# masafumiendo/benchnav

Measured on AMD Instinct MI355X. Metric: MPPI solve-steps/sec (K=1024,T=50,256x256 map), higher is better.
Workload: dtype f32

## Files before the change

### benchnav_amd/csrc/mppi_capi.cpp

```cpp
#include "../../include/benchnav_mppi.h"
#include "mppi_kernels.h"
#include "astar_dwa.h"

#include <algorithm>
#include <atomic>
#include <cmath>
#include <chrono>
#include <cstdarg>
#include <cstdio>
#include <cstdlib>
#include <cstring>
#include <cerrno>
#include <sys/stat.h>
#include <fcntl.h>
#include <sys/file.h>
#include <unistd.h>
#include <dlfcn.h>
#include <hsa/hsa.h>
#include <hsa/hsa_ext_amd.h>
#include <rccl/rccl.h>
#include <map>
#include <mutex>
#include <numeric>
#include <string>
#include <vector>

namespace {

constexpr int kProfGroup = 10;
bool wave_kernel_is_faster(const bn::SolveParams &p, size_t resident_role_wgs, int n_cus)
{
    const double W = (double)p.B * (p.nblk + 1), R = (double)std::max<size_t>(resident_role_wgs, 1), rows = std::max(0, p.nblk - 16);
    const double role = (4.5 + 0.19 * p.T + 0.3 * rows) * (1.0 + 0.175 * std::min(W, R) / std::max(n_cus, 1)) * std::max(1.0, W / R);
    const double gain = (rows == 0 && p.T >= 20) ? 0.93 : 1.0;
    const double wave = gain * (3.3 + 0.44 * p.T + 0.37 * rows) * (1.0 + 1.5 * W / (24.0 * std::max(n_cus, 1)));
    return wave < role;
}
thread_local std::string g_last_error;

#ifdef BN_EXPERIMENTS
inline const char *exp_env(const char *name) { return std::getenv(name); }
#else
inline const char *exp_env(const char *) { return nullptr; }
#endif

int fail(int code, const char *fmt, ...)
{
    char buf[512];
    va_list ap;
    va_start(ap, fmt);
    vsnprintf(buf, sizeof buf, fmt, ap);
    va_end(ap);
    g_last_error = buf;
    return code;
}

#define BN_HIP(expr)                                                                         \
    do {                                                                                     \
        hipError_t e_ = (expr);                                                              \
        if (e_ != hipSuccess) {                                                              \
            (void)hipGetLastError();    \
            return fail(BN_ERR_HIP, "%s failed: %s (%s:%d)", #expr, hipGetErrorString(e_),  \
                        __FILE__, __LINE__);                                                 \
        }                                                                                    \
    } while (0)

bool is_pow2_float(float v)
{
    int ex;
    return v > 0.0f && std::isfinite(v) && std::frexp(v, &ex) == 0.5f;
}

std::mutex g_overlap_mu;
std::map<int, bn_mppi *> g_overlap_owner;
std::map<int, std::vector<bn_mppi *>> g_handles;
std::atomic<int> g_overlap_owners{0};
std::map<int, int> g_overlap_lock_fd;
// ... 54 lines not shown
    hipStream_t xstream[kMaxStreams - 1] = {};
    std::vector<hipStream_t> parked;
    hipEvent_t ev_fork = nullptr, ev_join[kMaxStreams - 1] = {};
    hipEvent_t ev_guard[kMaxStreams] = {};
    unsigned long long *d_flags = nullptr;
    bool role_overlap = false;
    unsigned long long *d_gran[kSlots] = {};
    float *d_Xalt[kMaxStreams - 1] = {}, *d_Ualt[kMaxStreams - 1] = {};
    unsigned long long pub[kSlots] = {};
    unsigned long long tails = 0;
    bool prev_published = false;
    bool overlap_used = false;
    bool overlap_off = false;
    int *h_err = nullptr, *d_err = nullptr;
    unsigned long long *h_mail = nullptr, *d_mail = nullptr;
    float *d_mean_snap = nullptr;
    float *d_state_snaps = nullptr;
    size_t snap_cap = 0;
    size_t snap_slot = 0;
    bool arm_state_snap = false;
    struct BatchRec { int32_t n; const float *states; const float *eps; bn_noise_kind noise; int32_t eps_ring; int64_t eps_stride; bool episode; const float *z; };
    std::vector<BatchRec> journal;
    bool journal_lost = false;
    bool arm_snap = false;
    bool replaying = false, last_batch_overlapped = false;
    uint64_t journal_solves0 = 0, recoveries = 0;
    struct OvTune { double best[2] = {0, 0}, last[2] = {0, 0}, ema[2] = {0, 0}; int chosen = 0, explore = 0, slow_run = 0; uint64_t windows[2] = {0, 0}, since_explore = 0, switches = 0; } tune;
    struct OvSample { bool valid = false; std::chrono::steady_clock::time_point t{}; uint32_t prog = 0, enq = 0; } ov_sample;
    int run_mode = 0;
    float *self_out_copy = nullptr;
    const float *inline_state = nullptr;
    bool self_tail_launched = false;
    bool self_used = false;
    bool self_off = false;
    bool hp_enabled = false;
    hipStream_t hp_stream[2] = {};
    hipEvent_t hp_ev[2] = {};
    bool hp_unordered = false;
    int hp_unordered_q = 0;
    unsigned long long *h_req = nullptr, *d_req = nullptr;
    unsigned long long *req_bar = nullptr;
    unsigned long long *d_req_dev = nullptr;
    uint32_t hp_seq = 0;
    bool hp_armed = false;
    uint32_t hp_tag = 0;
    int hp_slot = 0, hp_q = 0, hp_xidx = 0;
    uint32_t hp_posted_tag = 0;
    float hp_posted_state[3] = {};
    float *hp_posted_out = nullptr;
    bool hp_skip_check = false;
    int hp_redo_q = -1;
    float hp_prev_state[3] = {};
    bool hp_gran_valid = false;
    int hp_extra = 2;
    int x_idx = 0;
    int hp_next_q = 0;
    std::chrono::steady_clock::time_point hp_armed_at{};
    int hp_polls = 25000;
    bool lat_kernel = false;
    bool wave_kernel = false;
    bool shard_pending = false;
    void *shard_comm = nullptr;
    int shard_world = 0, shard_rank = 0;
    bool shard_prepared = false;
    bool shard_inplace = false;
    float *d_gathered = nullptr;
// ... 304 lines not shown
    BN_HIP(hipStreamSynchronize(h->stream));
    h->recoveries += 1;
    (void)fail(BN_OK, "warning: an overlapped launch gave up waiting for its predecessor's partials; %zu batch(es) were re-run on one "
                      "stream (results are valid now; this handle no longer overlaps its launches)", recs.size());
    return BN_OK;
}

int settle_overlap(bn_mppi *h, bool synced)
{
    if (!h->overlap_used || h->replaying) return BN_OK;
    if (__atomic_load_n(h->h_err, __ATOMIC_ACQUIRE) == 0) {
        if (synced) {
            bool idle = true;
            for (int q = 0; idle && q + 1 < h->n_streams; ++q) idle = hipStreamQuery(h->xstream[q]) == hipSuccess;
            (void)hipGetLastError();
            if (idle) { h->overlap_used = false; h->journal.clear(); h->journal_lost = false; }
        }
        return BN_OK;
    }
    return recover_overlap(h);
}

int sync_checked(bn_mppi *h)
{
    BN_HIP(hipStreamSynchronize(h->stream));
    if (h->overlap_used)
        for (int q = 0; q + 1 < h->n_streams; ++q)
            if (h->xstream[q]) BN_HIP(hipStreamSynchronize(h->xstream[q]));
    return settle_overlap(h, true);
}

int self_check(bn_mppi *h)
{
    if (!h->self_used || h->overlap_used || h->replaying) return BN_OK;
    if (__atomic_load_n(h->h_err, __ATOMIC_ACQUIRE) == 0) return BN_OK;
    BN_HIP(hipStreamSynchronize(h->stream));
    BN_HIP(hipMemset(h->d_flags, 0, ((kSlots + 1) * (size_t)h->p.B + 3) * bn::kFlagStride * sizeof(unsigned long long)));
    for (int q = 0; q < kSlots; ++q) h->pub[q] = 0;
    h->tails = 0;
    *h->h_err = 0;
    h->self_used = false;
    h->self_off = true;
    return fail(BN_ERR_HIP, "the tail of a one-launch solve gave up waiting for the rollout workgroups of its own launch: the outputs of solve %llu "
                            "are invalid (solve again); this handle goes back to two launches per synchronous solve",
                (unsigned long long)h->solves - 1);
}

int settle_point(bn_mppi *h)
{
    hp_cancel(h);
    h->hp_gran_valid = false;
    if (int rc = self_check(h)) return rc;
    if (!h->overlap_used || h->replaying) return BN_OK;
    if (int rc = flush_tail(h)) return rc;
    return sync_checked(h);
}

void tune_record(bn_mppi *h, int mode, double us)
{
    bn_mppi::OvTune &t = h->tune;
    t.last[mode] = us;
    t.ema[mode] = t.ema[mode] == 0 ? us : t.ema[mode] + (us - t.ema[mode]) / 8;
    if (us >= 0.7 * t.ema[mode] && (t.best[mode] == 0 || us < t.best[mode])) t.best[mode] = us;
    t.windows[mode] += 1;
    if (mode == t.chosen) {
        t.since_explore += 1;
// ... 534 lines not shown
static int order_behind_foreign_overlap(bn_mppi *h, hipStream_t st)
{
    std::lock_guard<std::mutex> lock(g_overlap_mu);
    auto it = g_overlap_owner.find(h->cfg.device_id);
    if (it == g_overlap_owner.end() || it->second == h || !it->second) return BN_OK;
    bn_mppi *o = it->second;
    bool busy = false;
    for (int q = 0; q < o->n_streams; ++q) {
        const hipStream_t os = q ? o->xstream[q - 1] : o->stream;
        if (os == st || (q && !os)) continue;
        if (hipStreamQuery(os) == hipSuccess) continue;
        busy = true;
        if (!o->ev_guard[q]) continue;
        BN_HIP(hipEventRecord(o->ev_guard[q], os));
        BN_HIP(hipStreamWaitEvent(st, o->ev_guard[q], 0));
    }
    (void)hipGetLastError();
    if (!busy) { g_overlap_owner.erase(it); g_overlap_owners.store((int)g_overlap_owner.size(), std::memory_order_relaxed); }
    return BN_OK;
}

namespace {
int guard_foreign_overlap(bn_mppi *h)
{
    if (h->last_batch_overlapped || g_overlap_owners.load(std::memory_order_relaxed) == 0) return BN_OK;
    return order_behind_foreign_overlap(h, h->stream);
}
}

static inline bool lone_self_redo(const bn_mppi *h, bool self_tail, bool overlap)
{
    return h->hp_redo_q >= 0 && self_tail && !overlap && h->lat_kernel && !h->in_episode && !h->tail_pending && !h->replaying && !h->self_off &&
           !(h->cfg.flags & BN_FLAG_NO_PIPELINE);
}

static int solve_impl(bn_mppi_t *h, const float *states, bn_mem_kind states_where, const float *eps, bn_noise_kind noise,
                      bool shard_rollout, bool overlap = false, hipStream_t on_stream = nullptr, int alt_buffers = 0, bool self_tail = false)
{
    if (!h) return fail(BN_ERR_INVALID, "null handle");
    if (!states) return fail(BN_ERR_INVALID, "states is null");
    if (!h->map_set || !h->goal_set) return fail(BN_ERR_STATE, "set_map and set_goal must precede solve");
    if ((noise == BN_NOISE_PHILOX) != (eps == nullptr))
        return fail(BN_ERR_INVALID, "eps must be NULL exactly when noise == BN_NOISE_PHILOX");
    BN_BIND(h);
    hp_cancel(h);
    h->hp_gran_valid = false;
    if (!overlap && g_overlap_owners.load(std::memory_order_relaxed) > 0) {
        if (int rc = order_behind_foreign_overlap(h, on_stream ? on_stream : h->stream)) return rc;
    }

    bn::SolveParams p = h->p;
    const size_t B = p.B, K = p.K, T = p.T;
    h->map_epoch_at_solve = h->map_epoch;
    if (h->d_flags && (h->overlap_used || !h->journal.empty()))
        p.err_dev = reinterpret_cast<int *>(h->d_flags + ((kSlots + 1) * B + 2) * bn::kFlagStride);
    if (states_where == BN_MEM_DEVICE) {
        p.state = states;
    } else {
        if (h->solves) BN_HIP(hipStreamSynchronize(h->stream));
        std::memcpy(h->h_pinned, states, B * 3 * 4);
        BN_HIP(hipMemcpyAsync(h->d_state, h->h_pinned, B * 3 * 4, hipMemcpyHostToDevice, h->stream));
        p.state = h->d_state;
    }
    bn::EpsMode mode = bn::kEpsPhilox;
    switch (noise) {
    case BN_NOISE_PHILOX: break;
// ... 95 lines not shown
            h->self_tail_launched = true;
            h->prev_published = false;
            h->hp_gran_valid = p.gran != nullptr;
            h->x_idx = 0;
        } else
        if ((h->lat_kernel || h->role_overlap) && overlap) {
            p.flag_part = h->d_flags;
            p.err = h->d_err; p.err_dev = reinterpret_cast<int *>(h->d_flags + ((kSlots + 1) * B + 2) * bn::kFlagStride);
            if (h->arm_snap) { p.mean_snap = h->d_mean_snap; h->arm_snap = false; }
            p.cur_slot = cur3; p.prev_slot = prev3;
            p.wait_part = h->pub[prev3];
            p.gran = p.lat_kernel ? h->d_gran[cur3] : nullptr;
            if (alt_buffers) {
                if (h->d_Xalt[alt_buffers - 1]) p.X = h->d_Xalt[alt_buffers - 1];
                if (h->d_Ualt[alt_buffers - 1] && p.U) p.U = h->d_Ualt[alt_buffers - 1];
            }
            p.overlap = (h->prev_published && p.have_prev) ? 1 : 0;
            p.gran_prev = (p.overlap && p.lat_kernel) ? h->d_gran[prev3] : nullptr;
            if (on_stream) st = on_stream;
            if (p.overlap) h->overlap_used = true;
            h->pub[cur3] += (unsigned long long)p.nblk;
            h->prev_published = true;
            if (self_tail && p.lat_kernel && !h->in_episode) {
                p.self_tail = 1;
                p.wait_part_self = h->pub[cur3];
                p.wait_tail_self = h->tails;
                h->tails += 1;
            }
        } else {
            h->prev_published = false;
        }
        p.aux_prio = (!p.wave_kernel && (size_t)p.B * (p.nblk + 1) > h->resident_wgs) ? 1 : 0;
        if (!p.wave_kernel && !p.store_u) p.U = nullptr;
        if (p.self_tail) BN_HIP(bn::launch_rollout_lat_self(p, mode, st));
        else BN_HIP(bn::launch_rollout(p, mode, st));
        if (st != h->stream && lone_self) {
            BN_HIP(hipEventRecord(h->hp_ev[h->hp_redo_q], st));
            BN_HIP(hipStreamWaitEvent(h->stream, h->hp_ev[h->hp_redo_q], 0));
        }
        if (prof_grouped) h->prof_in_group = (h->prof_in_group + 1) % kProfGroup;
        h->solves += 1;
        h->x_idx = 0;
        h->tail_pending = !p.self_tail;
        if (p.self_tail) h->prev_published = false;
        if (lone_self) h->last_batch_overlapped = false;
        return BN_OK;
    }
    if (!(h->ticket_overlap && overlap && !shard_rollout)) h->prev_published = false;
    p.have_prev = 0;
    p.mean_from_part = 0;
    p.tail_solve = p.solve;
    if (p.slip_on && !h->slip_std_set) return fail(BN_ERR_STATE, "bn_mppi_set_slip_std must precede solve in sampled-slip mode");
    if (h->ticket_mode && !shard_rollout) {
        p.have_prev = h->tail_pending ? 1 : 0;
        p.tail_merged = 1;
        p.tail_solve = p.solve - 1;
        p.ustar_cur = h->d_ustar2[cur3]; p.stats_cur = h->d_stats2[cur3];
        p.ustar_prev = h->d_ustar2[prev3]; p.stats_prev = h->d_stats2[prev3];
        p.ticket = h->d_ticket;
        hipStream_t st = h->stream;
        p.flag_tail = h->d_flags + kSlots * B * bn::kFlagStride;
        if (p.have_prev) { p.wait_tail = h->tails; h->tails += 1; }
        if (h->ticket_overlap && overlap) {
            p.flag_part = h->d_flags;
            p.err = h->d_err; p.err_dev = reinterpret_cast<int *>(h->d_flags + ((kSlots + 1) * B + 2) * bn::kFlagStride);
            if (h->arm_snap) { p.mean_snap = h->d_mean_snap; h->arm_snap = false; }
            p.cur_slot = cur3; p.prev_slot = prev3;
            p.wait_part = h->pub[prev3];
            if (alt_buffers) {
                if (h->d_Xalt[alt_buffers - 1]) p.X = h->d_Xalt[alt_buffers - 1];
                if (h->d_Ualt[alt_buffers - 1] && p.U) p.U = h->d_Ualt[alt_buffers - 1];
            }
            p.overlap = (h->prev_published && p.have_prev) ? 1 : 0;
            if (on_stream) st = on_stream;
            if (p.overlap) h->overlap_used = true;
            h->pub[cur3] += 1;
            h->prev_published = true;
        }
        if (p.slip_on) BN_HIP(bn::launch_rollout_sampled(p, mode, st));
        else BN_HIP(bn::launch_rollout(p, mode, st));
        if (prof_grouped) h->prof_in_group = (h->prof_in_group + 1) % kProfGroup;
        h->solves += 1;
        h->tail_pending = true;
        return BN_OK;
    }
    if (shard_rollout && h->shard_inplace) p.part = h->d_gathered + (size_t)h->shard_rank * p.nblk * (2 + 2 * T);
    if (p.slip_on) {
        BN_HIP(bn::launch_rollout_sampled(p, mode, h->stream));
    } else {
        if (h->slow_path) p.wave_kernel = 1;
        else if (!p.store_u) p.U = nullptr;
        BN_HIP(bn::launch_rollout(p, mode, h->stream));
    }
    if (prof) BN_HIP(hipEventRecord(ev[1], h->stream));
    if (shard_rollout) {
        if (prof) BN_HIP(hipEventRecord(ev[2], h->stream));
        h->solves += 1;
        h->tail_pending = false;
        h->shard_pending = true;
        return BN_OK;
    }
    p.state = p.state_copy;
    BN_HIP(bn::launch_finish(p, h->stream));
    if (prof) BN_HIP(hipEventRecord(ev[2], h->stream));
    h->solves += 1;
    h->tail_pending = false;
    return BN_OK;
}

int bn_mppi_solve_async(bn_mppi_t *h, const float *states, bn_mem_kind states_where, const float *eps,
                        bn_noise_kind noise)
{
    if (h && !h->replaying && !h->journal.empty()) {
        h->last_batch_overlapped = false;
        journal_arm_states(h);
        journal_push(h, bn_mppi::BatchRec{1, states, eps, noise, 1, 0, false, nullptr}, states_where == BN_MEM_DEVICE && noise != BN_NOISE_HOST_KT2);
    }
    return solve_impl(h, states, states_where, eps, noise, false);
}

#ifdef BN_TIMING
struct HpClock { const char *name; long long ns = 0, n = 0; };
static HpClock g_hpc[6] = {{"post: request words"}, {"post: hipStreamWaitEvent"}, {"prelaunch: checks + ack"}, {"prelaunch: kernel launch"}, {"prelaunch: hipEventRecord"}, {"self_check + bind"}};
struct HpTick { int i; std::chrono::steady_clock::time_point t0 = std::chrono::steady_clock::now();
// ... 1287 lines not shown
```

### benchnav_amd/csrc/mppi_kernels.h

```cpp
#pragma once
#include <hip/hip_runtime.h>
#include <stdint.h>

namespace bn {

constexpr int kRolloutsPerBlock = 64;
constexpr int kRolloutThreads = 320;
constexpr int kChunk = 4;
constexpr int kWaveParkSteps = 30;
constexpr int kUPad = 65;
constexpr int kWideFinishThreads = 1024;
constexpr int kFinishThreads = kRolloutThreads;

enum EpsMode : int { kEpsPhilox = 0, kEpsKT2 = 1, kEpsT2K = 2 };

struct SolveParams {
    int K, T, G, B;
    int nblk;
    int Kp;
    int WN;
    int reach;
    int spec_extra;
    int map_stride;
    int pow2;
// ... 62 lines not shown
    int cur_slot, prev_slot;
    unsigned long long *flag_part;
    unsigned long long *flag_tail;
    unsigned long long wait_part;
    unsigned long long wait_tail;
    unsigned long long wait_part_self;
    unsigned long long wait_tail_self;
    int *err;
    int *err_dev;
    float *state_snap;
    float *mean_snap;
    unsigned long long *gran, *gran_prev;
    float *w;
    float *ustar;
    float *xstar;
    unsigned long long *mail;
    float *out_copy;
    float *stats;
    int trace_by_parity;
    unsigned long long *stamps;
    int ustar_written;
    float *out_copy_self;
    int host_paced;
    const unsigned long long *req_host;
    unsigned long long *req_dev;
    unsigned long long *spec_status;
    int req_direct;
    uint32_t req_tag;
    int req_polls;
    int no_early_mail;
    int aux_first;
    int state_inline;
    float sv0, sv1, sv2;
};

constexpr int kFlagStride = 32;

inline dim3 rollout_grid(const SolveParams &p, bool aux)
{
    const unsigned gx = (unsigned)p.nblk << p.xs;
    const unsigned rows = ((unsigned)p.B + (1u << p.xs) - 1) >> p.xs;
    const unsigned n_aux = (aux ? (unsigned)p.B : 0u) + (p.self_tail ? (unsigned)p.B : 0u);
    const unsigned aux_rows = (n_aux + gx - 1) / gx;
    return dim3(gx, rows + aux_rows);
}

size_t rollout_lds_bytes(const SolveParams &p);
size_t finish_lds_bytes(const SolveParams &p);
size_t finish_lds_bytes_for(SolveParams p, bool sampled);
size_t wave_lds_bytes(const SolveParams &p);
size_t lat_lds_bytes(const SolveParams &p);
int rollout_blocks_per_cu(const SolveParams &p);

hipError_t launch_rollout(const SolveParams &p, EpsMode mode, hipStream_t s);
hipError_t launch_rollout_lat_self(const SolveParams &p, EpsMode mode, hipStream_t s);
hipError_t launch_rollout_lat_host(const SolveParams &p, hipStream_t s, hipEvent_t stop);
hipError_t launch_rollout_lat_host_ref(const SolveParams &p, hipStream_t s, hipEvent_t stop);
hipError_t launch_finish(const SolveParams &p, hipStream_t s);
hipError_t launch_shard_merge(const SolveParams &p, float *group_rows, int *ticket, hipStream_t s);
hipError_t launch_reroll(const SolveParams &p, EpsMode mode, int b, const int *idx, int n, float *out_n_T1_3, hipStream_t s);
hipError_t launch_rollout_sampled(const SolveParams &p, EpsMode mode, hipStream_t s);
size_t sampled_resident_per_cu(const SolveParams &p);
bool sampled_fused(const SolveParams &p);
hipError_t launch_dwa(const SolveParams &p, const float *actions, const float *stage_goal, int NA, float *Xall, float *cost,
                      float *w, int *best, float *best_states, float *best_action, hipStream_t s);
hipError_t launch_dwa_window(const SolveParams &p, const float *prev_action, const float a_lim[2], float dwa_dt, int nv, int nw,
// ... 22 lines not shown
```

### benchnav_amd/csrc/mppi_kernels.hip

```cpp
#include "mppi_kernels.h"
#include "mppi_device.h"
#include "dwa_device.h"
#include <cstring>

namespace bn {

namespace {

template <int GEO, bool LDSWIN, int NT, bool REF>
__global__ __launch_bounds__(NT) void finish_kernel(const SolveParams p)
{
    extern __shared__ __attribute__((aligned(16))) float smem[];
    finish_body<GEO, LDSWIN, NT, true, false, true, REF>(p, blockIdx.x, p.part, p.cost, p.state, smem);
}

constexpr int kShardMergeThreads = 256;
__global__ __launch_bounds__(kShardMergeThreads) void shard_merge_kernel(const SolveParams p, float *grows, int *ticket)
{
    extern __shared__ __attribute__((aligned(16))) float smem[];
    const int T = p.T, tid = threadIdx.x, PS = 2 + 2 * p.T;
    float *us = smem, *sc = us + 2 * T, *red = sc + 64;
    int *flag = reinterpret_cast<int *>(red + 32);
    float m, S;
    if (p.nblk > 64) {
// ... 250 lines not shown
    return hipGetLastError();
}

template <int GEO, bool LDSWIN>
hipError_t launch_finish_t(const SolveParams &p, hipStream_t s)
{
    return p.ref_order ? launch_finish_r<GEO, LDSWIN, true>(p, s) : launch_finish_r<GEO, LDSWIN, false>(p, s);
}

}

size_t wave_lds_bytes(const SolveParams &p)
{
    const size_t wn_f = ((size_t)p.WN * p.WN + 3) & ~(size_t)3;
    const size_t own = std::max(wn_f + 4 * ((size_t)p.T + 1), (size_t)16 * kUPad + 4) + 2 * (size_t)p.T + 4 + 64 + (size_t)p.nblk + 32 + 4 +
                       (p.lds_park ? (size_t)16 * kUPad : 0);
#if defined(BN_EXPERIMENTS) && defined(BN_WAVE_LDS_PAD)
    return std::max(sizeof(float) * own, finish_lds_bytes(p) + 256) + BN_WAVE_LDS_PAD;
#endif
    return std::max(sizeof(float) * own, finish_lds_bytes(p) + 256);
}

size_t lat_lds_bytes(const SolveParams &p)
{
    if (p.WN <= 0) return 0;
    const size_t wcap = (size_t)p.WN + 2 * (size_t)p.spec_extra;
    const size_t own = ((size_t)p.T + 1) * 256 + 5 * 64 + 64 + 8 + wcap * wcap + 4 * (size_t)p.T + 2 * ((size_t)p.T + 2 * kChunk) * kUPad;
    const size_t bytes = std::max(sizeof(float) * own, finish_lds_bytes(p) + 256);
    return bytes <= 160 * 1024 ? bytes : 0;
}

size_t rollout_lds_bytes(const SolveParams &p)
{
    return sizeof(float) * ((size_t)p.WN * p.WN + 4 * (size_t)p.T + 2 * (size_t)p.T * kUPad + 2 * kChunk * 4 * 64 + 5 * 64 + 64);
}

size_t finish_lds_bytes(const SolveParams &p)
{
    const size_t slip = p.slip_on ? 2 * (size_t)p.WN * p.WN + (size_t)p.T + 16 : 0;
    const size_t groups = (p.nblk > 64 && p.nblk <= 64 * 16) ? (size_t)((p.nblk + 15) / 16) * (2 + 2 * (size_t)p.T) : 0;
    return sizeof(float) * ((size_t)p.WN * p.WN + 2 * (size_t)p.T + 3 * ((size_t)p.T + 1) + (size_t)p.nblk + 32 + groups + slip);
}

size_t finish_lds_bytes_for(SolveParams p, bool sampled)
{
    p.slip_on = sampled ? 1 : 0;
    return finish_lds_bytes(p);
}

hipError_t launch_rollout(const SolveParams &p, EpsMode mode, hipStream_t s)
{
    if (p.wave_kernel) return launch_rollout_wave(p, mode, s);
    if (p.ref_order)
        switch (mode) {
        case kEpsPhilox: return launch_rollout_role_ref_philox(p, s);
        case kEpsKT2: return launch_rollout_role_ref_kt2(p, s);
        default: return launch_rollout_role_ref_t2k(p, s);
        }
    switch (mode) {
    case kEpsPhilox: return launch_rollout_role_philox(p, s);
    case kEpsKT2: return launch_rollout_role_kt2(p, s);
    default: return launch_rollout_role_t2k(p, s);
    }
}

hipError_t launch_rollout_lat_self(const SolveParams &p, EpsMode mode, hipStream_t s)
{
// ... 230 lines not shown
```

### benchnav_amd/csrc/rollout_role.inc

```
#include "mppi_device.h"

#ifndef BN_ROLE_REF
#define BN_ROLE_REF false
#endif
#ifndef BN_ROLE_FRESH
#define BN_ROLE_FRESH false
#endif

namespace bn {

namespace {

template <int EPS, int GEO, bool LDSWIN, bool STORE_U, bool TICKET, bool REF>
__global__ __launch_bounds__(kRolloutThreads) void rollout_kernel(const SolveParams p)
{
    extern __shared__ __attribute__((aligned(16))) float smem[];
    BN_TRACE_BEGIN();
    const WgId wg = decode_wg(p);
    if (wg.idle) return;
    if (wg.aux) {
        if (p.aux_prio) __builtin_amdgcn_s_setprio(3);
        if (p.overlap) finish_body<GEO, LDSWIN, kRolloutThreads, false, true, false, REF>(p, wg.b, p.part_prev, p.cost_prev, p.state_prev, smem);
        else finish_body<GEO, LDSWIN, kRolloutThreads, false, false, false, REF>(p, wg.b, p.part_prev, p.cost_prev, p.state_prev, smem);
        BN_TRACE_END();
        return;
    }
    const int T = p.T, K = p.K;
    float *ring = smem;
    float *fin = ring + 2 * TU * 4 * 64;
    float *el = fin + 5 * 64;
    float *win = el + 64;
    float *ml = win + (LDSWIN ? p.WN * p.WN : 0);
    float *mv = ml + 2 * T;
    float *Ul = mv + 2 * T;

    const int tid = threadIdx.x;
    const int wid = tid >> 6, lane = tid & 63;
    const int wv = (wid == 0) ? 3 : (wid == 4) ? 4 : wid - 1;
    const int b = wg.b;
    const int k = wg.blk * kRolloutsPerBlock + lane;
    const bool active = k < K;
    const int kk = active ? k : K - 1;

    const float *__restrict__ map = p.map + (size_t)b * p.map_stride;
    const float *__restrict__ eps = p.eps;
    const float *st_src = p.closed_loop ? p.state_prev : p.state;
    float sx = st_src[b * 3 + 0], sy = st_src[b * 3 + 1], sth = st_src[b * 3 + 2];
    const float gx = p.goal[b * 2 + 0], gy = p.goal[b * 2 + 1];
    const uint64_t solve = p.solve;
    BN_STAMP(0);

    const float *part_prev = p.part_prev + (size_t)b * p.nblk * (2 + 2 * T);
    const bool ov = p.overlap && p.mean_from_part;
    MergeLoads pre{};
    const bool pre_ok = p.mean_from_part && p.nblk <= 64 && !ov;
    if (pre_ok) pre = merge_issue(part_prev, p.nblk, T, tid);

    Win w{0, 0, 0.f, 0.f, 0.f, 0.f};
    if (LDSWIN && !p.closed_loop) {
        w = window_origin<GEO>(p, sx, sy);
        stage_window(win, map, w, p.WN, p.G, tid, kRolloutThreads);
    }
    if (ov) {
        if (tid == 0) wait_counter<16>(flag_ctr(p.flag_part, p.prev_slot * p.B + b), p.wait_part, p);
        __syncthreads();
        if (p.closed_loop) {
            sx = load_agent(st_src + b * 3 + 0); sy = load_agent(st_src + b * 3 + 1); sth = load_agent(st_src + b * 3 + 2);
        }
        float m_unused, S_unused;
        merge_partials<kRolloutThreads, true>(part_prev, p.nblk, T, ml, ring, ring + p.nblk, tid, m_unused, S_unused, false, pre);
        for (int j = tid; j < 2 * T; j += kRolloutThreads) mv[j] = ml[j] * ((j & 1) ? p.iv1 : p.iv0);
// ... 1 lines not shown
        float m_unused, S_unused;
        merge_partials<kRolloutThreads>(part_prev, p.nblk, T, ml, ring, ring + p.nblk, tid, m_unused, S_unused, pre_ok, pre);
        for (int j = tid; j < 2 * T; j += kRolloutThreads) mv[j] = ml[j] * ((j & 1) ? p.iv1 : p.iv0);
    } else if (TICKET && p.overlap) {
        if (tid == 0) wait_counter<16>(flag_ctr(p.flag_part, p.prev_slot * p.B + b), p.wait_part, p);
        __syncthreads();
        for (int j = tid; j < 2 * T; j += kRolloutThreads) {
            const float m = load_agent(p.mean + (size_t)b * 2 * T + j);
            ml[j] = m;
            mv[j] = m * ((j & 1) ? p.iv1 : p.iv0);
        }
    } else {
        for (int j = tid; j < 2 * T; j += kRolloutThreads) {
            const float m = p.mean[(size_t)b * 2 * T + j];
            ml[j] = m;
            mv[j] = m * ((j & 1) ? p.iv1 : p.iv0);
        }
    }
    if (p.closed_loop) {
        const EnvStep e = env_advance<GEO>(p, b, sx, sy, sth, ml[0], ml[1], p.env_z, (uint64_t)p.ep_index);
        sx = e.x; sy = e.y; sth = e.th;
        if (LDSWIN) {
            w = window_origin<GEO>(p, sx, sy);
            stage_window(win, map, w, p.WN, p.G, tid, kRolloutThreads);
        }
    }
    const bool pub = !TICKET && p.flag_part != nullptr;
    const bool tpub = TICKET && p.flag_part != nullptr;
    if (wg.blk == 0 && tid == 0) {
        if (pub || (TICKET && p.flag_part != nullptr)) { store_agent(p.state_copy + b * 3 + 0, sx); store_agent(p.state_copy + b * 3 + 1, sy); store_agent(p.state_copy + b * 3 + 2, sth); }
        else { p.state_copy[b * 3 + 0] = sx; p.state_copy[b * 3 + 1] = sy; p.state_copy[b * 3 + 2] = sth; }
        if (p.state_snap) { p.state_snap[b * 3 + 0] = sx; p.state_snap[b * 3 + 1] = sy; p.state_snap[b * 3 + 2] = sth; }
    }
    BN_BAR();
    if (p.mean_snap && wg.blk == 0 && wid == 0) snapshot_mean(p, b, ml, lane);

    const size_t Kp = (size_t)p.Kp;
    const bool lean = p.lean != 0;
    float *Xb = p.X + (size_t)b * (T + 1) * 3 * Kp + k;
    float *Ub = STORE_U ? p.U + (size_t)b * T * 2 * Kp + k : nullptr;

    if (wid < 4) {
#pragma unroll
        for (int q = 0; q < TU / 4; ++q) {
            const int t = wid * (TU / 2) + 2 * q;
            if (t < T) produce_pair<EPS, STORE_U, BN_ROLE_FRESH>(p, eps, b, kk, t, solve, ml, Ul, Ub, Kp, lane);
        }
    }
    BN_BAR();
    BN_STAMP(1);

    Chain c;
    double Sd = 0.0, Ad = 0.0;
    float th_a = sth;
    if (wv == 0) {
        c.x = sx; c.y = sy; c.th = sth;
        sincos_spec(c.th, c.sn, c.cs);
        c.trav = trav_lookup<GEO, LDSWIN, true>(p, win, map, w, c.x, c.y);
    }

#define BN_CHAIN(FIRST, i, slot)                                                                               \
    do {                                                                                                       \
        float xn, yn, dth;                               \
        if constexpr (REF) chain_step<GEO, LDSWIN, FIRST, true, false, 0, true>(p, win, map, w, c, uc[i][0], uc[i][1], xn, yn, dth);    \
        else chain_step<GEO, LDSWIN, FIRST, false, true>(p, win, map, w, c, uc[i][0], uc[i][1], xn, yn, dth,   \
                                                    i + 1 < TU ? uc[(i + 1) % TU][0] : un[0][0], i + 1 < TU ? uc[(i + 1) % TU][1] : un[0][1]);   \
// ... 35 lines not shown
                __builtin_amdgcn_sched_barrier(0);                                                             \
                _Pragma("unroll") for (int i = 0; i < TU; ++i) {                                               \
                    const int t = (cc) * TU + i;                                                               \
                    if (!(GUARD) || t < T) {                                                                   \
                        if ((FIRSTCHUNK) && i == 0) BN_CHAIN(true, i, slot + i * 256);                         \
                        else BN_CHAIN(false, i, slot + i * 256);                                               \
                    }                                                                                          \
                }                                                                                              \
                _Pragma("unroll") for (int i = 0; i < TU; ++i) { uc[i][0] = un[i][0]; uc[i][1] = un[i][1]; }   \
            }                                                                                                  \
        } else if (wv >= 3) {                                                                                  \
            if ((cc) >= 1) {                                                                                   \
                const float *slot = ring + ((((cc) - 1) & 1) * TU) * 256;                                      \
                float4 rq[TU];                              \
                _Pragma("unroll") for (int i = 0; i < TU; ++i)                                                 \
                    rq[i] = reinterpret_cast<const float4 *>(slot + i * 256)[lane];                            \
                _Pragma("unroll") for (int i = 0; i < TU; ++i) {                                               \
                    const int t = ((cc) - 1) * TU + i;                                                         \
                    if (!(GUARD) || t < T) {                                                                   \
                        if (wv == 3) BN_CONSUME_A(t, rq[i]);                                                   \
                        else BN_CONSUME_B(t, rq[i]);                                                           \
                    }                                                                                          \
                }                                                                                              \
            }                                                                                                  \
        } else {                                                                                               \
            _Pragma("unroll") for (int q = 0; q < TU / 4; ++q) {                                               \
                const int t = ((cc) + 2) * TU + (wv == 1 ? 0 : TU / 2) + 2 * q;                                \
                if (t < T) produce_pair<EPS, STORE_U, BN_ROLE_FRESH>(p, eps, b, kk, t, solve, ml, Ul, Ub, Kp, lane);          \
            }                                                                                                  \
        }                                                                                                      \
    } while (0)

    const int nfull = T / TU;
    float uc[TU][2];
    if (wv == 0) {
#pragma unroll
        for (int i = 0; i < TU; ++i) {
            const int t = min(i, T - 1);
            uc[i][0] = Ul[(2 * t) * kUPad + lane];
            uc[i][1] = Ul[(2 * t + 1) * kUPad + lane];
        }
        if constexpr (!REF) chain_prepare(p, c, uc[0][0], uc[0][1]);
    }
    BN_PHASE(0, true, true);
    BN_BAR();
    BN_STAMP(2);
    int cc = 1;
    BN_TIMING_DO(
    unsigned long long busy = 0;
    )
    for (; cc < nfull; ++cc) {
        BN_TIMING_DO(
        const unsigned long long t_a = __builtin_readcyclecounter();
        )
        BN_PHASE(cc, false, false);
        BN_TIMING_DO(
        busy += __builtin_readcyclecounter() - t_a;
        )
        BN_BAR();
    }
    BN_TIMING_DO(
    if (p.stamps && blockIdx.x == 0 && blockIdx.y == 0 && lane == 0) p.stamps[16 + wv] = busy;
    )
    for (; cc * TU < T + TU; ++cc) {
        BN_PHASE(cc, false, true);
        BN_BAR();
    }
#undef BN_PHASE
#undef BN_CONSUME_A
#undef BN_CONSUME_B
#undef BN_CHAIN
    BN_STAMP(3);

    if (wv == 0) {
        fin[lane] = c.x; fin[64 + lane] = c.y; fin[192 + lane] = c.trav;
        if constexpr (REF) fin[128 + lane] = c.th;
    } else if (wv == 3) {
        fin[256 + lane] = (float)Ad;
    }
    BN_BAR();

    if (wv == 3) {
        if (!lean) {
            float *Xt = Xb + (size_t)(3 * T) * Kp;
            Xt[0] = fin[lane]; Xt[Kp] = fin[64 + lane]; Xt[2 * Kp] = REF ? fin[128 + lane] : th_a;
        }
    } else if (wv == 4) {
        const float xT = fin[lane], yT = fin[64 + lane], trT = fin[192 + lane], A = fin[256 + lane];
        const float dxT = xT - gx, dyT = yT - gy;
        const float term = sqrt_cr_normal(dxT * dxT + dyT * dyT) + (trT <= p.thr ? 1.0e4f : 0.0f);
        const float cost = ((float)Sd + term) + A;
        if (active) { if (pub || tpub) store_agent(p.cost + (size_t)b * K + k, cost); else p.cost[(size_t)b * K + k] = cost; }
        const float z = active ? (-cost) / p.lambda_ : -INFINITY;
        const float zmax = wave_max(z);
        const float e = active ? expf(z - zmax) : 0.0f;
        const float esum = wave_sum(e);
        el[lane] = e;
        if (lane == 0) {
            float *part = p.part + ((size_t)b * p.nblk + wg.blk) * (2 + 2 * T);
            if (TICKET || pub) { store_agent(part, zmax); store_agent(part + 1, esum); }
            else { part[0] = zmax; part[1] = esum; }
        }
    }
    BN_BAR();
    BN_STAMP(4);
    if (!TICKET && pub) {
        column_sums<kRolloutThreads, true>(Ul, el, T, tid, p.part + ((size_t)b * p.nblk + wg.blk) * (2 + 2 * T));
        publish_counter(flag_ctr(p.flag_part, p.cur_slot * p.B + b), tid);
    } else {
        column_sums<kRolloutThreads, TICKET>(Ul, el, T, tid, p.part + ((size_t)b * p.nblk + wg.blk) * (2 + 2 * T));
    }
    BN_STAMP(5);
    if (TICKET) ticket_merge<kRolloutThreads>(p, b, wg.blk, smem);
    BN_TRACE_END();
}

template <int EPS, int GEO, bool LDSWIN, bool STORE_U>
hipError_t launch_rollout_u(const SolveParams &p, hipStream_t s)
{
    const dim3 grid = rollout_grid(p, p.have_prev != 0);
    const size_t lds = rollout_lds_bytes(p);
    if (p.ticket) {
        hipError_t e = ensure_lds(rollout_kernel<EPS, GEO, LDSWIN, STORE_U, true, BN_ROLE_REF>, lds);
        if (e != hipSuccess) return e;
        rollout_kernel<EPS, GEO, LDSWIN, STORE_U, true, BN_ROLE_REF><<<grid, dim3(kRolloutThreads), lds, s>>>(p);
    } else {
        hipError_t e = ensure_lds(rollout_kernel<EPS, GEO, LDSWIN, STORE_U, false, BN_ROLE_REF>, lds);
        if (e != hipSuccess) return e;
        rollout_kernel<EPS, GEO, LDSWIN, STORE_U, false, BN_ROLE_REF><<<grid, dim3(kRolloutThreads), lds, s>>>(p);
    }
    return hipGetLastError();
}

template <int EPS, int GEO, bool LDSWIN>
hipError_t launch_rollout_t(const SolveParams &p, hipStream_t s)
{
    return p.U ? launch_rollout_u<EPS, GEO, LDSWIN, true>(p, s) : launch_rollout_u<EPS, GEO, LDSWIN, false>(p, s);
}

template <int EPS>
hipError_t launch_rollout_e(const SolveParams &p, hipStream_t s)
{
    const bool win = p.WN > 0;
    switch (geo_of(p)) {
    case kGeoPow2Origin0: return win ? launch_rollout_t<EPS, kGeoPow2Origin0, true>(p, s) : launch_rollout_t<EPS, kGeoPow2Origin0, false>(p, s);
    case kGeoPow2: return win ? launch_rollout_t<EPS, kGeoPow2, true>(p, s) : launch_rollout_t<EPS, kGeoPow2, false>(p, s);
    default: return win ? launch_rollout_t<EPS, kGeoGeneral, true>(p, s) : launch_rollout_t<EPS, kGeoGeneral, false>(p, s);
    }
}


}

}

#include "rollout_lat.inc"

namespace bn {

hipError_t BN_ROLE_LAUNCHER(const SolveParams &p, hipStream_t s)
{
    if (p.lat_kernel) return launch_lat_e<BN_ROLE_EPS>(p, s);
    return launch_rollout_e<BN_ROLE_EPS>(p, s);
}

#ifdef BN_ROLE_OCCUPANCY
int rollout_blocks_per_cu(const SolveParams &p)
{
    int n = 0;
    const size_t lds = rollout_lds_bytes(p);
    if (hipOccupancyMaxActiveBlocksPerMultiprocessor(&n, rollout_kernel<kEpsPhilox, kGeoPow2Origin0, true, false, false, false>, kRolloutThreads, lds) != hipSuccess) return -1;
    return n;
}

#endif

}
```

Before: 108,400.

## Replace workgroup barriers in role rollout kernel with LDS progress-counter handoffs

Adds a CTR variant of the role-split rollout kernel in which the chain, producer and consumer waves synchronise through LDS progress counters with s_sleep polling instead of workgroup-wide barriers per chunk. Waves can then run ahead of each other, so the chain wave no longer stalls at each phase barrier. The variant is on by default for the non-wave, non-latency paths. It adds bounded spin-waits with an error flag and host-side error reporting, and it adds a small amount of LDS.

New measurement: 105,800. 2.4% lower.

```diff
diff --git a/benchnav_amd/csrc/mppi_capi.cpp b/benchnav_amd/csrc/mppi_capi.cpp
--- a/benchnav_amd/csrc/mppi_capi.cpp
+++ b/benchnav_amd/csrc/mppi_capi.cpp
@@ -43,6 +43,15 @@
 #else
 inline const char *exp_env(const char *) { return nullptr; }
 #endif
+
+bool role_counter_loop(const bn::SolveParams &, int)
+{
+#ifdef BN_ROLE_CTR_FORCE
+    return BN_ROLE_CTR_FORCE != 0;
+#endif
+    if (const char *e = exp_env("BN_ROLE_CTR")) return e[0] != '0';
+    return true;
+}
 
 int fail(int code, const char *fmt, ...)
 {
@@ -163,6 +172,7 @@
     const float *inline_state = nullptr;
     bool self_tail_launched = false;
     bool self_used = false;
+    bool role_ctr_used = false;
     bool self_off = false;
     bool hp_enabled = false;
     hipStream_t hp_stream[2] = {};
@@ -533,6 +543,12 @@
 
 int self_check(bn_mppi *h)
 {
+    if (h->role_ctr_used && !h->overlap_used && !h->replaying && !h->self_used && __atomic_load_n(h->h_err, __ATOMIC_ACQUIRE) != 0) {
+        BN_HIP(hipStreamSynchronize(h->stream));
+        *h->h_err = 0;
+        return fail(BN_ERR_HIP, "a wave of the rollout kernel gave up waiting for a hand-off inside its workgroup: the outputs of the solves "
+                                "since the last synchronisation point are invalid");
+    }
     if (!h->self_used || h->overlap_used || h->replaying) return BN_OK;
     if (__atomic_load_n(h->h_err, __ATOMIC_ACQUIRE) == 0) return BN_OK;
     BN_HIP(hipStreamSynchronize(h->stream));
@@ -1133,6 +1149,14 @@
 {
     return h->hp_redo_q >= 0 && self_tail && !overlap && h->lat_kernel && !h->in_episode && !h->tail_pending && !h->replaying && !h->self_off &&
            !(h->cfg.flags & BN_FLAG_NO_PIPELINE);
+}
+
+static inline void role_loop_for(bn_mppi *h, bn::SolveParams &p)
+{
+    p.role_ctr = role_counter_loop(p, h->n_cus) ? 1 : 0;
+    if (!p.role_ctr) return;
+    if (!p.err) p.err = h->d_err;
+    h->role_ctr_used = true;
 }
 
 static int solve_impl(bn_mppi_t *h, const float *states, bn_mem_kind states_where, const float *eps, bn_noise_kind noise,
@@ -1294,6 +1318,7 @@
         }
         p.aux_prio = (!p.wave_kernel && (size_t)p.B * (p.nblk + 1) > h->resident_wgs) ? 1 : 0;
         if (!p.wave_kernel && !p.store_u) p.U = nullptr;
+        if (!p.wave_kernel && !p.lat_kernel) role_loop_for(h, p);
         if (p.self_tail) BN_HIP(bn::launch_rollout_lat_self(p, mode, st));
         else BN_HIP(bn::launch_rollout(p, mode, st));
         if (st != h->stream && lone_self) {
@@ -1340,7 +1365,7 @@
             h->prev_published = true;
         }
         if (p.slip_on) BN_HIP(bn::launch_rollout_sampled(p, mode, st));
-        else BN_HIP(bn::launch_rollout(p, mode, st));
+        else { role_loop_for(h, p); BN_HIP(bn::launch_rollout(p, mode, st)); }
         if (prof_grouped) h->prof_in_group = (h->prof_in_group + 1) % kProfGroup;
         h->solves += 1;
         h->tail_pending = true;
@@ -1352,6 +1377,7 @@
     } else {
         if (h->slow_path) p.wave_kernel = 1;
         else if (!p.store_u) p.U = nullptr;
+        if (!p.wave_kernel) role_loop_for(h, p);
         BN_HIP(bn::launch_rollout(p, mode, h->stream));
     }
     if (prof) BN_HIP(hipEventRecord(ev[1], h->stream));
diff --git a/benchnav_amd/csrc/mppi_kernels.h b/benchnav_amd/csrc/mppi_kernels.h
--- a/benchnav_amd/csrc/mppi_kernels.h
+++ b/benchnav_amd/csrc/mppi_kernels.h
@@ -118,6 +118,7 @@
     int aux_first;
     int state_inline;
     float sv0, sv1, sv2;
+    int role_ctr;
 };
 
 constexpr int kFlagStride = 32;
diff --git a/benchnav_amd/csrc/mppi_kernels.hip b/benchnav_amd/csrc/mppi_kernels.hip
--- a/benchnav_amd/csrc/mppi_kernels.hip
+++ b/benchnav_amd/csrc/mppi_kernels.hip
@@ -306,7 +306,7 @@
 
 size_t rollout_lds_bytes(const SolveParams &p)
 {
-    return sizeof(float) * ((size_t)p.WN * p.WN + 4 * (size_t)p.T + 2 * (size_t)p.T * kUPad + 2 * kChunk * 4 * 64 + 5 * 64 + 64);
+    return sizeof(float) * ((size_t)p.WN * p.WN + 4 * (size_t)p.T + 2 * (size_t)p.T * kUPad + 2 * kChunk * 4 * 64 + 5 * 64 + 64 + 8);
 }
 
 size_t finish_lds_bytes(const SolveParams &p)
diff --git a/benchnav_amd/csrc/rollout_role.inc b/benchnav_amd/csrc/rollout_role.inc
--- a/benchnav_amd/csrc/rollout_role.inc
+++ b/benchnav_amd/csrc/rollout_role.inc
@@ -7,11 +7,42 @@
 #define BN_ROLE_FRESH false
 #endif
 
+#ifndef BN_ROLE_SLEEP_CC
+#define BN_ROLE_SLEEP_CC 2
+#endif
+#ifndef BN_ROLE_SLEEP_CP
+#define BN_ROLE_SLEEP_CP 1
+#endif
+#ifndef BN_ROLE_SLEEP_FC
+#define BN_ROLE_SLEEP_FC 2
+#endif
+
 namespace bn {
 
 namespace {
 
-template <int EPS, int GEO, bool LDSWIN, bool STORE_U, bool TICKET, bool REF>
+typedef __attribute__((address_space(3))) volatile int role_vint;
+typedef int role_i2 __attribute__((ext_vector_type(2)));
+typedef __attribute__((address_space(3))) volatile role_i2 role_vint2;
+constexpr int kRoleWaitCap = 1 << 20;
+
+__device__ __forceinline__ void role_wait_expired(const SolveParams &p, int what)
+{
+    if (p.err) raise_wait_expired(p, nullptr, (unsigned long long)what);
+}
+
+template <int SLEEP>
+__device__ __forceinline__ void role_wait_ge(role_vint *ctr, int need, const SolveParams &p, int what)
+{
+    for (int it = 0; it < kRoleWaitCap; ++it) {
+        if (*ctr >= need) { asm volatile("" ::: "memory"); return; }
+        __builtin_amdgcn_s_sleep(SLEEP);
+    }
+    role_wait_expired(p, what);
+    asm volatile("" ::: "memory");
+}
+
+template <int EPS, int GEO, bool LDSWIN, bool STORE_U, bool TICKET, bool REF, bool CTR>
 __global__ __launch_bounds__(kRolloutThreads) void rollout_kernel(const SolveParams p)
 {
     extern __shared__ __attribute__((aligned(16))) float smem[];
@@ -29,14 +60,15 @@
     float *ring = smem;
     float *fin = ring + 2 * TU * 4 * 64;
     float *el = fin + 5 * 64;
-    float *win = el + 64;
+    int *prog = reinterpret_cast<int *>(el + 64);
+    float *win = el + 64 + 8;
     float *ml = win + (LDSWIN ? p.WN * p.WN : 0);
     float *mv = ml + 2 * T;
     float *Ul = mv + 2 * T;
 
     const int tid = threadIdx.x;
     const int wid = tid >> 6, lane = tid & 63;
-    const int wv = (wid == 0) ? 3 : (wid == 4) ? 4 : wid - 1;
+    const int wv = CTR ? ((0x24103 >> (4 * wid)) & 7) : ((wid == 0) ? 3 : (wid == 4) ? 4 : wid - 1);
     const int b = wg.b;
     const int k = wg.blk * kRolloutsPerBlock + lane;
     const bool active = k < K;
@@ -104,6 +136,7 @@
         else { p.state_copy[b * 3 + 0] = sx; p.state_copy[b * 3 + 1] = sy; p.state_copy[b * 3 + 2] = sth; }
         if (p.state_snap) { p.state_snap[b * 3 + 0] = sx; p.state_snap[b * 3 + 1] = sy; p.state_snap[b * 3 + 2] = sth; }
     }
+    if constexpr (CTR) { if (tid < 8) prog[tid] = tid == 2 ? 1 : (tid == 4 && p.lean) ? (1 << 30) : 0; }
     BN_BAR();
     if (p.mean_snap && wg.blk == 0 && wid == 0) snapshot_mean(p, b, ml, lane);
 
@@ -205,6 +238,7 @@
     } while (0)
 
     const int nfull = T / TU;
+    if constexpr (!CTR) {
     float uc[TU][2];
     if (wv == 0) {
 #pragma unroll
@@ -239,10 +273,6 @@
         BN_PHASE(cc, false, true);
         BN_BAR();
     }
-#undef BN_PHASE
-#undef BN_CONSUME_A
-#undef BN_CONSUME_B
-#undef BN_CHAIN
     BN_STAMP(3);
 
     if (wv == 0) {
@@ -277,6 +307,222 @@
     }
     BN_BAR();
     BN_STAMP(4);
+    } else {
+    role_vint *cprog = (role_vint *)prog;
+    role_vint *pprog = cprog + 1;
+#define BN_RSTAMP(i, v) BN_TIMING_DO(if (p.stamps && blockIdx.x == 0 && blockIdx.y == 0 && lane == 0) p.stamps[8000 + 16 * wv + (i)] = (v);)
+    BN_TIMING_DO(unsigned long long n_wait_p = 0; unsigned long long n_wait_c = 0;)
+    BN_RSTAMP(0, __builtin_readcyclecounter());
+    const int nchunk = (T + TU - 1) / TU;
+    const int rem = T - nfull * TU;
+    float cost_b = 0.0f;
+    if (wv == 0) {
+#define BN_CLOAD(U, cn)                                                                                        \
+    _Pragma("unroll") for (int i = 0; i < TU; ++i) {                                                           \
+        const int t_ = min((cn) * TU + i, T - 1);                                                              \
+        U[i][0] = Ul[(2 * t_) * kUPad + lane];                                                                 \
+        U[i][1] = Ul[(2 * t_ + 1) * kUPad + lane];                                                             \
+    }
+#define BN_CSTEP(FIRST, UC, UN, i, slotp)                                                                      \
+    do {                                                                                                       \
+        float xn, yn, dth;                                                                                     \
+        if constexpr (REF) chain_step<GEO, LDSWIN, FIRST, true, false, 0, true>(p, win, map, w, c, UC[i][0], UC[i][1], xn, yn, dth);   \
+        else chain_step<GEO, LDSWIN, FIRST, false, true>(p, win, map, w, c, UC[i][0], UC[i][1], xn, yn, dth,   \
+                                                    i + 1 < TU ? UC[(i + 1) % TU][0] : UN[0][0], i + 1 < TU ? UC[(i + 1) % TU][1] : UN[0][1]);   \
+        __builtin_amdgcn_sched_barrier(0);                                                                     \
+        reinterpret_cast<float4 *>(slotp)[lane] = make_float4(xn, yn, dth, c.trav);      \
+    } while (0)
+#define BN_CCHUNK(UC, UN, ccv, PAR, FIRSTCHUNK, NS, GUARD, CHECKC)                                             \
+    do {                                                                                                       \
+        float *slot = ring + ((PAR) * TU) * 256;                                                               \
+        const int have = pprog[1 - (PAR)];                                                                     \
+        asm volatile("" ::: "memory");                                                                         \
+        BN_CLOAD(UN, (ccv) + 1)                                                                                \
+        __builtin_amdgcn_sched_barrier(0);                                                                     \
+        role_i2 cab = {0, 0};                                                                                  \
+        _Pragma("unroll") for (int i = 0; i < (NS); ++i) {                                                     \
+            if ((CHECKC) && i == (NS) - 1) { cab = *(role_vint2 *)(cprog + 4); asm volatile("" ::: "memory"); __builtin_amdgcn_sched_barrier(0); } \
+            if (!(GUARD) || (ccv) * TU + i < T) {                                                              \
+                if ((FIRSTCHUNK) && i == 0) BN_CSTEP(true, UC, UN, i, slot + i * 256);                         \
+                else BN_CSTEP(false, UC, UN, i, slot + i * 256);                                               \
+            }                                                                                                  \
+        }                                                                                                      \
+        asm volatile("" ::: "memory");                                                                         \
+        if (!(GUARD) && (NS) == TU) *cprog = ((ccv) + 1) * TU;    \
+        if (((ccv) + 1) * TU < T && __builtin_amdgcn_readfirstlane(have) < (ccv) + 1) {                        \
+            BN_TIMING_DO(++n_wait_p;)                                                                          \
+            role_wait_ge<BN_ROLE_SLEEP_CP>(pprog + (1 - (PAR)), (ccv) + 1, p, 1);                              \
+            BN_CLOAD(UN, (ccv) + 1)                                                                            \
+            if constexpr (!REF) chain_prepare(p, c, UN[0][0], UN[0][1]);    \
+        }                                                                                                      \
+        if (CHECKC) {                                                                                          \
+            BN_TIMING_DO(if (__builtin_amdgcn_readfirstlane(min(cab.x, cab.y)) < (ccv) * TU) ++n_wait_c;)      \
+            if (__builtin_amdgcn_readfirstlane(cab.x) < (ccv) * TU) role_wait_ge<BN_ROLE_SLEEP_CC>(cprog + 4, (ccv) * TU, p, 2);   \
+            if (__builtin_amdgcn_readfirstlane(cab.y) < (ccv) * TU) role_wait_ge<BN_ROLE_SLEEP_CC>(cprog + 5, (ccv) * TU, p, 3);   \
+        }                                                                                                      \
+    } while (0)
+        float ua[TU][2], ub[TU][2];
+        BN_CLOAD(ua, 0)
+        if constexpr (!REF) chain_prepare(p, c, ua[0][0], ua[0][1]);
+        if (nfull > 0) BN_CCHUNK(ua, ub, 0, 0, true, TU, false, false);
+        else BN_CCHUNK(ua, ub, 0, 0, true, TU, true, false);
+        BN_STAMP(2);
+        int cc = 1;
+        for (; cc + 1 < nfull; cc += 2) {
+            BN_CCHUNK(ub, ua, cc, 1, false, TU, false, true);
+            BN_CCHUNK(ua, ub, cc + 1, 0, false, TU, false, true);
+        }
+        if (cc < nfull) {
+            BN_CCHUNK(ub, ua, cc, 1, false, TU, false, true);
+#pragma unroll
+            for (int i = 0; i < TU; ++i) { ub[i][0] = ua[i][0]; ub[i][1] = ua[i][1]; }
+            ++cc;
+        }
+        if (rem && nfull > 0) {
+            const int par = cc & 1;
+            if (rem == 1) BN_CCHUNK(ub, ua, cc, par, false, 1, false, false);
+            else if (rem == 2) BN_CCHUNK(ub, ua, cc, par, false, 2, false, false);
+            else BN_CCHUNK(ub, ua, cc, par, false, 3, false, false);
+        }
+#undef BN_CCHUNK
+#undef BN_CSTEP
+#undef BN_CLOAD
+        reinterpret_cast<float4 *>(ring + (T & (2 * TU - 1)) * 256)[lane] = make_float4(c.x, c.y, REF ? c.th : 0.0f, c.trav);
+        asm volatile("" ::: "memory");
+        *cprog = T + 1;
+        BN_STAMP(3);
+        BN_RSTAMP(1, __builtin_readcyclecounter()); BN_RSTAMP(2, n_wait_p); BN_RSTAMP(3, n_wait_c);
+    } else if (wv <= 2) {
+        for (int cc = 1 + wv; cc < nchunk; cc += 2) {
+#pragma unroll
+            for (int q = 0; q < TU / 2; ++q) {
+                const int t = cc * TU + 2 * q;
+                if (t < T) produce_pair<EPS, STORE_U, BN_ROLE_FRESH>(p, eps, b, kk, t, solve, ml, Ul, Ub, Kp, lane);
+            }
+            asm volatile("" ::: "memory");
+            pprog[cc & 1] = cc;
+        }
+        BN_RSTAMP(1, __builtin_readcyclecounter());
+        if (wv == 2) {
+            const int last = nchunk - 1;
+            if (last >= 2) role_wait_ge<BN_ROLE_SLEEP_FC>(pprog + (last & 1), last, p, 6);
+            if (last >= 3) role_wait_ge<BN_ROLE_SLEEP_FC>(pprog + ((last - 1) & 1), last - 1, p, 7);
+            int t = 0;
+            for (; t + 4 <= T; t += 4) {
+                float u[8], q[8];
+#pragma unroll
+                for (int i = 0; i < 8; ++i) { u[i] = Ul[(2 * t + i) * kUPad + lane]; q[i] = mv[2 * t + i]; }
+#pragma unroll
+                for (int i = 0; i < 4; ++i) Ad += (double)(p.lambda_ * (q[2 * i] * u[2 * i] + q[2 * i + 1] * u[2 * i + 1]));
+            }
+            for (; t < T; ++t) {
+                const float u0 = Ul[(2 * t) * kUPad + lane], u1 = Ul[(2 * t + 1) * kUPad + lane];
+                const float a = mv[2 * t] * u0 + mv[2 * t + 1] * u1;
+                Ad += (double)(p.lambda_ * a);
+            }
+            fin[256 + lane] = (float)Ad;
+            asm volatile("" ::: "memory");
+            cprog[3] = 1;
+            BN_RSTAMP(2, __builtin_readcyclecounter());
+        }
+    } else if (wv == 4 || !lean) {
+        role_vint *mine = cprog + (wv == 3 ? 4 : 5);
+        const float4 *rbase = reinterpret_cast<const float4 *>(ring) + lane;
+        float *Xt = Xb;
+        float term = 0.0f;
+        int t = 0, idle = 0, pr;
+        float4 rq[TU];
+#define BN_LOOK_AT(tt)                                                                                         \
+    do {                                                                                                       \
+        const float4 *sl_ = rbase + 64 * ((tt) & TU);                                                          \
+        pr = *cprog;                                                                                           \
+        asm volatile("" ::: "memory");                                                                         \
+        _Pragma("unroll") for (int i = 0; i < TU; ++i) rq[i] = sl_[64 * i];                                    \
+        asm volatile("" :: "v"(rq[0].z), "v"(rq[1].z), "v"(rq[2].z), "v"(rq[3].z));    \
+    } while (0)
+#define BN_STEP_A(o, first)                                                                                    \
+    do {                                                                                                       \
+        Xt[0] = o.x; Xt[Kp] = o.y; Xt[2 * Kp] = REF ? o.z : theta_step(th_a, o.z, first);    \
+        Xt += 3 * Kp;                                                                                          \
+    } while (0)
+        BN_LOOK_AT(0);
+        while (t <= T) {
+            int n = min(__builtin_amdgcn_readfirstlane(pr), T + 1) - t;
+            if (n <= 0) {
+                if (++idle < kRoleWaitCap) { __builtin_amdgcn_s_sleep(BN_ROLE_SLEEP_FC); BN_LOOK_AT(t); continue; }
+                role_wait_expired(p, 4);
+                n = T + 1 - t;
+            }
+            n = min(n, TU);
+            float4 cur[TU];
+#pragma unroll
+            for (int i = 0; i < TU; ++i) cur[i] = rq[i];
+            asm volatile("" ::: "memory");
+            *mine = t + n;
+            asm volatile("" ::: "memory");
+            BN_LOOK_AT(t + n);
+            __builtin_amdgcn_sched_barrier(0);
+            if (wv == 3) {
+                if (n == TU && t + TU <= T) {
+#pragma unroll
+                    for (int i = 0; i < TU; ++i) BN_STEP_A(cur[i], t + i == 0);
+                } else {
+#pragma unroll
+                    for (int i = 0; i < TU; ++i) {
+                        if (i < n && t + i < T) BN_STEP_A(cur[i], t + i == 0);
+                        else if (i < n) {
+                            Xt[0] = cur[i].x; Xt[Kp] = cur[i].y; Xt[2 * Kp] = REF ? cur[i].z : th_a;
+                        }
+                    }
+                }
+            } else {
+                if (n == TU && t + TU <= T) {
+#pragma unroll
+                    for (int i = 0; i < TU; ++i) BN_CONSUME_B(t + i, cur[i]);
+                } else {
+#pragma unroll
+                    for (int i = 0; i < TU; ++i) {
+                        if (i < n && t + i < T) BN_CONSUME_B(t + i, cur[i]);
+                        else if (i < n) {
+                            const float dxT = cur[i].x - gx, dyT = cur[i].y - gy;
+                            term = sqrt_cr_normal(dxT * dxT + dyT * dyT) + (cur[i].w <= p.thr ? 1.0e4f : 0.0f);
+                        }
+                    }
+                }
+            }
+            t += n;
+        }
+#undef BN_STEP_A
+#undef BN_LOOK_AT
+        BN_RSTAMP(1, __builtin_readcyclecounter()); BN_RSTAMP(2, (unsigned long long)idle);
+        if (wv == 4) {
+            role_wait_ge<BN_ROLE_SLEEP_FC>(cprog + 3, 1, p, 5);
+            const float A = fin[256 + lane];
+            const float cost = ((float)Sd + term) + A;
+            cost_b = cost;
+            const float z = !active ? -INFINITY : p.inv_lambda != 0.0f ? (-cost) * p.inv_lambda : (-cost) / p.lambda_;
+            const float zmax = wave_max(z);
+            const float e = active ? expf(z - zmax) : 0.0f;
+            const float esum = wave_sum(e);
+            el[lane] = e;
+            if (lane == 0) {
+                float *part = p.part + ((size_t)b * p.nblk + wg.blk) * (2 + 2 * T);
+                if (TICKET || pub) { store_agent(part, zmax); store_agent(part + 1, esum); }
+                else { part[0] = zmax; part[1] = esum; }
+            }
+        }
+    }
+    BN_RSTAMP(4, __builtin_readcyclecounter());
+    BN_BAR();
+    BN_RSTAMP(5, __builtin_readcyclecounter());
+#undef BN_RSTAMP
+    if (wv == 4 && active) { if (pub || tpub) store_agent(p.cost + (size_t)b * K + k, cost_b); else p.cost[(size_t)b * K + k] = cost_b; }
+    BN_STAMP(4);
+    }
+#undef BN_PHASE
+#undef BN_CONSUME_A
+#undef BN_CONSUME_B
+#undef BN_CHAIN
     if (!TICKET && pub) {
         column_sums<kRolloutThreads, true>(Ul, el, T, tid, p.part + ((size_t)b * p.nblk + wg.blk) * (2 + 2 * T));
         publish_counter(flag_ctr(p.flag_part, p.cur_slot * p.B + b), tid);
@@ -288,21 +534,24 @@
     BN_TRACE_END();
 }
 
+template <int EPS, int GEO, bool LDSWIN, bool STORE_U, bool TICKET, bool CTR>
+hipError_t launch_rollout_k(const SolveParams &p, hipStream_t s, dim3 grid, size_t lds)
+{
+    hipError_t e = ensure_lds(rollout_kernel<EPS, GEO, LDSWIN, STORE_U, TICKET, BN_ROLE_REF, CTR>, lds);
+    if (e != hipSuccess) return e;
+    rollout_kernel<EPS, GEO, LDSWIN, STORE_U, TICKET, BN_ROLE_REF, CTR><<<grid, dim3(kRolloutThreads), lds, s>>>(p);
+    return hipGetLastError();
+}
+
 template <int EPS, int GEO, bool LDSWIN, bool STORE_U>
 hipError_t launch_rollout_u(const SolveParams &p, hipStream_t s)
 {
     const dim3 grid = rollout_grid(p, p.have_prev != 0);
     const size_t lds = rollout_lds_bytes(p);
-    if (p.ticket) {
-        hipError_t e = ensure_lds(rollout_kernel<EPS, GEO, LDSWIN, STORE_U, true, BN_ROLE_REF>, lds);
-        if (e != hipSuccess) return e;
-        rollout_kernel<EPS, GEO, LDSWIN, STORE_U, true, BN_ROLE_REF><<<grid, dim3(kRolloutThreads), lds, s>>>(p);
-    } else {
-        hipError_t e = ensure_lds(rollout_kernel<EPS, GEO, LDSWIN, STORE_U, false, BN_ROLE_REF>, lds);
-        if (e != hipSuccess) return e;
-        rollout_kernel<EPS, GEO, LDSWIN, STORE_U, false, BN_ROLE_REF><<<grid, dim3(kRolloutThreads), lds, s>>>(p);
-    }
-    return hipGetLastError();
+    if (p.ticket) return p.role_ctr ? launch_rollout_k<EPS, GEO, LDSWIN, STORE_U, true, true>(p, s, grid, lds)
+                                    : launch_rollout_k<EPS, GEO, LDSWIN, STORE_U, true, false>(p, s, grid, lds);
+    return p.role_ctr ? launch_rollout_k<EPS, GEO, LDSWIN, STORE_U, false, true>(p, s, grid, lds)
+                      : launch_rollout_k<EPS, GEO, LDSWIN, STORE_U, false, false>(p, s, grid, lds);
 }
 
 template <int EPS, int GEO, bool LDSWIN>
@@ -342,7 +591,7 @@
 {
     int n = 0;
     const size_t lds = rollout_lds_bytes(p);
-    if (hipOccupancyMaxActiveBlocksPerMultiprocessor(&n, rollout_kernel<kEpsPhilox, kGeoPow2Origin0, true, false, false, false>, kRolloutThreads, lds) != hipSuccess) return -1;
+    if (hipOccupancyMaxActiveBlocksPerMultiprocessor(&n, rollout_kernel<kEpsPhilox, kGeoPow2Origin0, true, false, false, false, false>, kRolloutThreads, lds) != hipSuccess) return -1;
     return n;
 }
 
```
